# giladfrid009/WTracker

Hardware: AMD Instinct MI355X
Metric: frames/sec YOLOv8s+ResMLP sim loop @640x640 (higher is better)
Workload: dtype f16x3; 1 GPU; BASELINE configs[2]: full sim loop, YOLOv8s (nc=1, seeded synthetic weights) + ResMLP(imaging-100ms_pred-40ms_moving-50ms, reference weights); batch_per_gpu=64, lanes_per_gpu=2, global_batch=64, headline_mode=f16x3, parallelism=single GPU

## Files before the change

### wtracker_amd/_build.py

```python
from __future__ import annotations

import os
import subprocess
import sys

PKG_DIR = os.path.dirname(os.path.abspath(__file__))
CSRC = os.path.join(PKG_DIR, "csrc")
LIB_PATH = os.path.join(PKG_DIR, "libwtk_hip.so")
SOURCES = ["wtk_api.hip", "wtk_plan.hip", "wtk_run.hip", "wtk_hybrid.hip", "conv_igemm.hip", "conv_sk.hip", "conv1x1_wide.hip", "conv3x3_halo.hip", "conv3x3_c32.hip", "front_fused.hip", "front_fused_split.hip", "c2f_fused.hip", "stem_pool.hip", "head.hip", "mlp.hip", "track_ops.hip", "comm.hip", "eval_ops.hip"]
HEADERS = ["wtk_kernels.h", "wtk_internal.h", os.path.join("..", "..", "include", "wtk_hip.h")]


def _hipcc() -> str:
    for cand in (os.environ.get("HIPCC"), "/opt/rocm/bin/hipcc", "hipcc"):
        if cand and (os.path.isabs(cand) and os.path.exists(cand) or not os.path.isabs(cand)):
            return cand
    return "hipcc"


BASE_FLAGS = ["--offload-arch=gfx950", "-O3", "-fPIC", "-std=c++17", "-ffp-contract=off", "-Wall", "-Wno-unused-function"]
STAMP = os.path.join(CSRC, ".flags")


def _flags() -> list:
# ... 86 lines not shown
```

### wtracker_amd/csrc/conv3x3_halo.hip

```cpp
#include "wtk_kernels.h"

#include <cstdlib>
#include <type_traits>

namespace wtk {

typedef _Float16 half8 __attribute__((ext_vector_type(8)));
typedef float floatx4 __attribute__((ext_vector_type(4)));

namespace {

template <typename T> struct ElemH;
template <> struct ElemH<_Float16> {
    static constexpr int CE = 8;
};
template <> struct ElemH<float> {
    static constexpr int CE = 4;
};

__device__ __forceinline__ float silu_h(float x) {
    return wtk_silu_scaled(x);
}

__device__ __forceinline__ void mma_h(const uint4 &wf, const uint4 &pf, floatx4 &acc, _Float16 *) {
// ... 127 lines not shown
    const bool ok = halo_out_coords(a, o_first + lane, xs, n, y, x);
    col_e = xs + x;
    pix_e = ok ? (n * a.H + y) * a.W + col_e : -1;
}
__device__ __forceinline__ int lane_fetch(int src_lane, int v) { return __builtin_amdgcn_ds_bpermute(src_lane * 4, v); }

template <typename T, int BN, int NHALO, int MINW, int NWB, int HROWS, int BMT = 256, bool TAIL = false, bool SPLIT = false>
__global__ __launch_bounds__(512, MINW) void conv3x3_halo_kernel(const HaloArgs a) {
    static_assert(!SPLIT || (sizeof(T) == 2 && BN != 192 && (MINW <= 2 || (BN == 64 && BMT == 128 && NHALO == 1))),
                  "split mode: fp16 storage, 64 / 128 couts, 256-register budget (128 for the two-blocks-per-CU form: 64 couts x 128 pixels, one window buffer)");
#ifdef WTK_HALO_STAMPS
    const unsigned long long st_t0 = __builtin_amdgcn_s_memrealtime();
#endif
    asm volatile("" ::"s"(a.in), "s"(a.w), "s"(a.bias), "s"(a.zeros), "s"(a.in_ld), "s"(a.in_coff), "s"(a.N), "s"(a.H), "s"(a.W), "s"(a.Cin), "s"(a.CoutPad),
                 "s"(a.Kpad), "s"(a.S), "s"(a.pitch), "s"(a.strips), "s"(a.d_strips.mul), "s"(a.d_strips.sh1), "s"(a.d_strips.sh2), "s"(a.d_pitch.mul),
                 "s"(a.d_pitch.sh1), "s"(a.d_pitch.sh2), "s"(a.d_nct.mul), "s"(a.d_nct.sh1), "s"(a.d_nct.sh2), "s"(a.d_h1.mul), "s"(a.d_h1.sh1), "s"(a.d_h1.sh2), "s"(a.grid), "s"(a.live_off));
    constexpr int CE = ElemH<T>::CE;
    constexpr int CCH = 8 * CE;
    constexpr int WAVES_C = BN == 64 ? 1 : 2, WAVES_P = 8 / WAVES_C;
    constexpr int WC = BN / WAVES_C;
    constexpr int WP = BMT / WAVES_P, TP = WP / 16, TC = WC / 16, NV = 4 * TC;
    constexpr int WR = BN / 64;

    constexpr int kHaloBytesT = HROWS * 128;
    __shared__ __attribute__((aligned(16))) char halo0[kHaloBytesT];
    __shared__ __attribute__((aligned(16))) char halo1[NHALO == 2 ? kHaloBytesT : 16];
    static_assert(NWB == 2 || NWB == 3 || (NWB == 6 && NHALO == 2 && !TAIL && SPLIT), "slab ring: 2, 3 or 6 (split tiles, two window buffers, no fused tail)");
    constexpr bool kRing = NWB >= 3;
    __shared__ __attribute__((aligned(16))) char wbuf0[NWB > 3 ? 16 : BN * 128];
    __shared__ __attribute__((aligned(16))) char wbuf1[NWB > 3 ? 16 : BN * 128];
    __shared__ __attribute__((aligned(16))) char wbuf2[NWB == 3 ? BN * 128 : 16];
// ... 13 lines not shown
        if ((int)blockIdx.x >= live) return;
        nwg = min(nwg, live);
    }
    int L;
    {
        const int bid = blockIdx.x;
        const int xcd = bid & 7, q = nwg >> 3, r = nwg & 7;
        L = (xcd < r ? xcd * (q + 1) : r * (q + 1) + (xcd - r) * q) + (bid >> 3);
    }
    const unsigned t = fdiv((unsigned)L, a.d_nct);
    const int n0 = (L - (int)t * nct) * BN;
    const int rb = (int)fdiv(t, a.d_strips);
    const int strip = (int)t - rb * a.strips;
    const int o0 = rb * BMT;
    const char *zero_page = reinterpret_cast<const char *>(a.zeros);
    if (a.live_off) {
        const unsigned u = (unsigned)strip * (unsigned)a.live_ld + ((unsigned)o0 >> 7);
        const unsigned wd = *reinterpret_cast<const unsigned *>(zero_page + a.live_off + (u & ~3u));
        if (((wd >> ((u & 3u) * 8)) & (BMT == 256 ? 0xffffu : 0xffu)) == 0) return;
    }
    const int xs = strip * a.S;
    const int pitch = a.pitch;
    const int halo_rows = BMT + 2 * pitch + 2;
    const int halo_pieces = (halo_rows + 7) >> 3;
    const int n_base = (int)fdiv(fdiv((unsigned)o0, a.d_pitch), a.d_h1);

    const T *in = reinterpret_cast<const T *>(a.in) + (long long)n_base * a.H * a.W * a.in_ld + a.in_coff;
    const T *wgt = reinterpret_cast<const T *>(a.w);

    constexpr int kMaxPiecesPerWave = (HROWS / 8 + 7) / 8;
    unsigned hoff[kMaxPiecesPerWave];
    unsigned hvalid;
    halo_piece_offsets<T, kMaxPiecesPerWave>(a, o0, xs, n_base, halo_rows, wave, lane, hoff, hvalid);
    const char *img = reinterpret_cast<const char *>(in);
    auto issue_halo_piece = [&](char *buf, int q, int c) {
// ... 1442 lines not shown
    a.d_bps = make_fastdiv((unsigned)a.blocks_per_strip);
    a.d_strips = make_fastdiv((unsigned)a.strips);
    a.d_pitch = make_fastdiv((unsigned)a.pitch);
    a.d_h1 = make_fastdiv((unsigned)(a.H + 1));
    const long long cap = num_cus / 8 * 8;
    const unsigned grid = (unsigned)(tiles < cap ? tiles : cap);
    a.grid = (int)grid;
    hipLaunchKernelGGL((conv3x3_halo_pkernel<T, BN, HROWS>), dim3(grid), dim3(512), 0, stream, a);
    return hipGetLastError();
}

template <typename T, int BN, int NHALO, int MINW, int NWB, int HROWS, int BMT = 256, bool TAIL = false, bool SPLIT = false> hipError_t launch_h(HaloArgs a, hipStream_t stream) {
    const long long blocks = (long long)a.strips * a.blocks_per_strip * (a.CoutPad / BN);
    if (blocks <= 0 || blocks > 0x7fffffffLL) return hipErrorInvalidValue;
    if (BMT + 2 * a.pitch + 2 > HROWS || (long long)a.blocks_per_strip * BMT < (long long)a.N * (a.H + 1) * a.pitch) return hipErrorInvalidValue;
    if (a.live_off && ((a.live_off & 3u) || (a.live_ld & 1) || (long long)a.live_ld * 128 < (long long)a.blocks_per_strip * BMT)) return hipErrorInvalidValue;
    a.d_nct = make_fastdiv((unsigned)(a.CoutPad / BN));
    a.d_bps = make_fastdiv((unsigned)a.blocks_per_strip);
    a.d_strips = make_fastdiv((unsigned)a.strips);
    a.d_pitch = make_fastdiv((unsigned)a.pitch);
    a.d_h1 = make_fastdiv((unsigned)(a.H + 1));
    a.grid = (int)blocks;
    hipLaunchKernelGGL((conv3x3_halo_kernel<T, BN, NHALO, MINW, NWB, HROWS, BMT, TAIL, SPLIT>), dim3((unsigned)blocks), dim3(512), 0, stream, a);
    return hipGetLastError();
}

}

bool halo_eligible(int k, int stride, int cin, int is_f16) {
    const int cch = is_f16 ? 64 : 32;
    return k == 3 && stride == 1 && cin % cch == 0;
// ... 154 lines not shown
```

### wtracker_amd/csrc/head.hip

```cpp
#include "wtk_kernels.h"

namespace wtk {

template <typename T> __device__ __forceinline__ float ldf(const T *p) { return (float)*p; }

constexpr int kStatusNonFinite = 1;
__device__ __forceinline__ bool not_finite(float x) { return !(fabsf(x) <= 3.402823466e+38f); }

__device__ __forceinline__ void better(float &s, int &i, float s2, int i2) {
    if (s2 > s || (s2 == s && i2 < i)) {
        s = s2;
        i = i2;
    }
}

template <typename T>
__device__ __forceinline__ bool head_scan(const HeadArgs &a, int n, float &best, int &best_i, float &best_l, float &second) {
    const int A0 = a.lh[0] * a.lw[0], A1 = a.lh[1] * a.lw[1], A2 = a.lh[2] * a.lw[2];
    const int A = A0 + A1 + A2;

    best = -INFINITY, best_l = -INFINITY, second = -INFINITY;
    best_i = 0x7fffffff;
    bool bad = false;
    auto merge = [](float &b, int &bi, float &bl, float &s2nd, float b2, int bi2, float bl2, float s2) __attribute__((always_inline)) {
// ... 139 lines not shown
    head_row<T>(a, n, keep, best_i, score);
}

template <typename T>
__global__ __launch_bounds__(1024) void head_select_kernel_sparse(const HeadSparseArgs q) {
    const HeadArgs &a = q.h;
    const int n = blockIdx.x;
    float best, best_l, second;
    int best_i;
    if (!head_scan<T>(a, n, best, best_i, best_l, second)) return;
    if (threadIdx.x != 0) return;
    if (a.out_margin) a.out_margin[n] = fminf(best_l - second, fabsf(best_l - a.conf_logit));
    const bool keep = (best_i != 0x7fffffff) && (best > a.conf);
    q.sel_anchor[n] = keep ? best_i : -1;
    q.sel_score[n] = best;
    if (!keep || (q.n_dyn && n >= *q.n_dyn)) return;
    const int A0 = a.lh[0] * a.lw[0], A1 = a.lh[1] * a.lw[1];
    const int lvl = best_i < A0 ? 0 : (best_i < A0 + A1 ? 1 : 2);
    const int j = best_i - (lvl == 0 ? 0 : (lvl == 1 ? A0 : A0 + A1));
    const int H = a.lh[lvl], W = a.lw[lvl], S = q.S[lvl], pitch = q.pitch[lvl], ld = q.ld[lvl];
    const int y = j / W, x = j % W;
    unsigned char *live0 = q.live + q.off0[lvl], *live1 = q.live + q.off1[lvl];
    for (int dy = -1; dy <= 1; ++dy)
        for (int dx = -1; dx <= 1; ++dx) {
            const int yy = y + dy, xx = x + dx;
            if (yy < 0 || yy >= H || xx < 0 || xx >= W) continue;
            const int s = xx / S;
            const int u = s * ld + (((n * (H + 1) + yy) * pitch + (xx - s * S)) >> 7);
            live0[u] = 1;
            if (dy == 0 && dx == 0) live1[u] = 1;
        }
}

template <typename T>
__global__ __launch_bounds__(64) void head_decode_kernel(const HeadSparseArgs q) {
    const int n = blockIdx.x;
    const int best_i = q.sel_anchor[n];
    head_row<T>(q.h, n, best_i >= 0, best_i, q.sel_score[n]);
}

constexpr float kNmsMaxWh = 7680.f;

template <typename T> __device__ __forceinline__ void decode_anchor(const HeadArgs &a, int n, int lvl, int j, int Al, float (&xyxy)[4]) {
    const T *b = reinterpret_cast<const T *>(a.box[lvl]) + ((long long)n * Al + j) * 64;
    float dist[4];
#pragma unroll
// ... 133 lines not shown
    }
    if (threadIdx.x == 0 && q.out_count) q.out_count[n] = count;
}

hipError_t launch_head_nms(const NmsArgs &a, int is_f16, hipStream_t stream) {
    if (a.h.N <= 0 || a.h.nc < 1 || a.h.cls_ld < a.h.nc || a.max_det < 1 || !a.scratch_score || !a.scratch_cls || !a.scratch_box || !a.out_xywh)
        return hipErrorInvalidValue;
    if (is_f16)
        hipLaunchKernelGGL((head_nms_kernel<_Float16>), dim3(a.h.N), dim3(1024), 0, stream, a);
    else
        hipLaunchKernelGGL((head_nms_kernel<float>), dim3(a.h.N), dim3(1024), 0, stream, a);
    return hipGetLastError();
}

hipError_t launch_head_select_sparse(const HeadSparseArgs &a, hipStream_t stream) {
    if (a.h.N <= 0 || a.h.nc < 1 || a.h.cls_ld < a.h.nc || !a.live || !a.sel_anchor || !a.sel_score) return hipErrorInvalidValue;
    hipLaunchKernelGGL((head_select_kernel_sparse<float>), dim3(a.h.N), dim3(1024), 0, stream, a);
    return hipGetLastError();
}
hipError_t launch_head_decode(const HeadSparseArgs &a, hipStream_t stream) {
    if (a.h.N <= 0 || !a.sel_anchor || !a.sel_score || !a.h.out_xywh) return hipErrorInvalidValue;
    hipLaunchKernelGGL((head_decode_kernel<float>), dim3(a.h.N), dim3(64), 0, stream, a);
    return hipGetLastError();
}

hipError_t launch_head(const HeadArgs &a, int is_f16, hipStream_t stream) {
    if (a.N <= 0 || a.nc < 1 || a.cls_ld < a.nc) return hipErrorInvalidValue;
    if (is_f16)
        hipLaunchKernelGGL((head_select_kernel<_Float16>), dim3(a.N), dim3(1024), 0, stream, a);
    else
        hipLaunchKernelGGL((head_select_kernel<float>), dim3(a.N), dim3(1024), 0, stream, a);
// ... 5 lines not shown
```

### wtracker_amd/csrc/wtk_internal.h

```cpp
#pragma once
#include "../../include/wtk_hip.h"
#include "wtk_kernels.h"

#include <cstring>
#include <map>
#include <mutex>
#include <string>
#include <utility>
#include <vector>

namespace wtk {
int fail(const std::string &msg);
int fail_hip(const char *what, hipError_t e);
int ensure_attributes(int device);
}
#define HIP_TRY(expr)                                                                                                          \
    do {                                                                                                                       \
        hipError_t _e = (expr);                                                                                                \
        if (_e != hipSuccess) return wtk::fail_hip(#expr, _e);                                                                 \
    } while (0)

struct DeviceGuard {
    int prev = -1;
    bool switched = false;
// ... 123 lines not shown
    int *nms_cls = nullptr;
    int use_halo = 1;
    int front_debug = 0;
    int use_tail = 1;
    int use_tail_cls_split = 1;
    int halo_small_blocks = 1;
    int halo_persist = 1;
    int halo_slabs = 3;
    int use_c32s = 1;
    int use_s2win = 1;
    int use_ws64 = 1;
    int use_wide = 1;
    int use_c2f = 0;
    int use_front = 0;
    int use_sparse_box = 1;
    struct DetLevel {
        int op0 = -1, box1 = -1, box2 = -1;
    } det[3];
    size_t live_bytes = 0;
    int *sel_anchor = nullptr;
    float *sel_score = nullptr;
    int sparse_B = 0;
    ConvLaunch sparse_done[6];
    int num_cus = 0;
    int latency = 0;
    int sk_group = 1;
    int sk_force_tile = -1, sk_force_form = -1;
    std::map<long long, wtk::SkChoice> sk_choices;
    int sk_autotune = 1;
    int tune_pass = -1;
    std::map<long long, std::vector<wtk::SkChoice>> sk_cands;
    std::map<long long, std::vector<float>> tune_ms;
    std::vector<hipEvent_t> tune_ev;
    std::vector<long long> tune_key;
// ... 31 lines not shown
```

### wtracker_amd/csrc/wtk_kernels.h

```cpp
#pragma once
#include <hip/hip_runtime.h>
#include <stdint.h>

namespace wtk {

struct FastDiv {
    unsigned mul, sh1, sh2;
};
inline FastDiv make_fastdiv(unsigned d) {
    FastDiv f;
    if (d == 0) d = 1;
    unsigned l = 0;
    while ((1ull << l) < d) ++l;
    const unsigned long long m = ((1ull << 32) * ((1ull << l) - d)) / d + 1;
    f.mul = (unsigned)m;
    f.sh1 = l < 1 ? l : 1;
    f.sh2 = l > 0 ? l - 1 : 0;
    return f;
}
__device__ __forceinline__ unsigned fdiv(unsigned n, const FastDiv &f) {
    const unsigned t = __umulhi(n, f.mul);
    return (t + ((n - t) >> f.sh1)) >> f.sh2;
}

// ... 197 lines not shown
    int S, pitch, strips, blocks_per_strip;
    const void *zeros;
    unsigned long long *dbg_stamps;
    const void *tail_w;
    const float *tail_bias;
    void *tail_out;
    int tail_kpad, tail_ld, tail_coff;
    int tail_cout;
    int tail_f32;
    int bm;
    int persist_cus;
    int slabs;
    int deep;
    int narrow;
    int grid;
    unsigned live_off;
    const int *n_dyn;
    FastDiv d_bps, d_strips, d_pitch, d_nct, d_h1;
    int live_ld;
};
static_assert(sizeof(HaloArgs) == 288, "live_off / live_ld fill padding: the struct of a dense launch is what it was before the live mask");
bool halo_eligible(int k, int stride, int cin, int is_f16);
bool split_halo_eligible(int k, int stride, int cin, int cout);
int split_halo_cout_tile(int cout_stored);
hipError_t launch_conv3x3_halo_split(const HaloArgs &a, hipStream_t stream);
bool split_s2win_eligible(int k, int stride, int cin, int cout, int cout_pad, int wo, bool plain);
hipError_t launch_conv3x3_s2_split(const HaloArgs &a, hipStream_t stream);
int halo_rows_max(int cout_stored, int slabs);
void halo_geometry(int H, int W, int rows_max, int *S, int *pitch, int *strips, int *blocks_per_strip, int bm = 256);
void halo_geometry_stacked(int N, int H, int W, int rows_max, int *S, int *pitch, int *strips, int *blocks_per_strip, int bm = 256);
int halo_cout_tile(int cout_stored);
hipError_t launch_conv3x3_halo(const HaloArgs &a, int is_f16, hipStream_t stream);
bool s2win_eligible(int k, int stride, int cin, int cout, int cout_pad, int is_f16, int wo, bool plain);
hipError_t launch_conv3x3_s2(const HaloArgs &a, hipStream_t stream);
int ws64_rows_max();
bool ws64_eligible(int k, int stride, int cin, int cout, int cout_pad, int is_f16, bool has_out2, bool has_tail);
// ... 115 lines not shown
    int N;
    float conf;
    float gain, pad_x, pad_y;
    float img_w, img_h;
    float *out_xywh;
    float *out_conf;
    int *out_anchor;
    float *out_margin;
    float conf_logit;
    int *status;
};
hipError_t launch_head(const HeadArgs &a, int is_f16, hipStream_t stream);

struct HeadSparseArgs {
    HeadArgs h;
    unsigned char *live;
    int *sel_anchor;
    float *sel_score;
    int S[3], pitch[3], ld[3];
    unsigned off0[3], off1[3];
    const int *n_dyn;
};
hipError_t launch_head_select_sparse(const HeadSparseArgs &a, hipStream_t stream);
hipError_t launch_head_decode(const HeadSparseArgs &a, hipStream_t stream);

struct NmsArgs {
    HeadArgs h;
    float iou;
    int max_det;
    float *scratch_score;
    int *scratch_cls;
    float *scratch_box;
    float *out_xywh;
    float *out_conf;
    int *out_cls;
    int *out_anchor;
    int *out_count;
};
hipError_t launch_head_nms(const NmsArgs &a, int is_f16, hipStream_t stream);
// ... 111 lines not shown
```

### wtracker_amd/csrc/wtk_plan.hip

```cpp
#include <execinfo.h>
#include <signal.h>
#include <unistd.h>

#include "wtk_internal.h"

#include <algorithm>
#include <cmath>
#include <cstdio>
#include <cstdlib>

using namespace wtk;

namespace {
static int make_divisible8(double x) { return (int)(std::ceil(x / 8.0) * 8.0); }

static ModelDims model_dims(float width, float depth, int max_ch, int nc) {
    ModelDims d;
    const int base[5] = {64, 128, 256, 512, 1024};
    for (int i = 0; i < 5; ++i) d.c[i] = make_divisible8(std::min(base[i], max_ch) * (double)width);
    const int nb[4] = {3, 6, 6, 3};
    for (int i = 0; i < 4; ++i) d.n[i] = std::max((int)std::lround(nb[i] * (double)depth), 1);
    d.hb = std::max(std::max(16, d.c[2] / 4), 64);
    d.hc = std::max(d.c[2], std::min(nc, 100));
    d.nc = nc;
// ... 311 lines not shown
    h->halo_persist = env_int("WTK_HALO_PERSIST", 1) != 0;
    h->halo_small_blocks = env_int("WTK_HALO_SMALL_BLOCKS", 1) != 0;
    h->use_tail = env_int("WTK_NO_FUSED_TAIL", 0) != 1;
    h->use_tail_cls_split = env_int("WTK_NO_SPLIT_CLS_TAIL", 0) != 1;
    h->use_wide = env_int("WTK_NO_WIDE_1X1", 0) != 1;
    h->use_ws64 = env_int("WTK_NO_WS64", 0) != 1;
    h->use_s2win = env_int("WTK_NO_S2WIN", 0) != 1;
    h->use_c32s = env_int("WTK_NO_C32S", 0) != 1;
    h->sk_group = env_int("WTK_SK_GROUP", 1) != 0;
    h->sk_autotune = env_int("WTK_SK_AUTOTUNE", 1) != 0;
    const int tile = env_int("WTK_SK_TILE", -1), form = env_int("WTK_SK_FORM", -1);
    h->sk_force_tile = tile >= 0 && tile <= 3 ? tile : -1;
    h->sk_force_form = form == 0 || form == 1 ? form : -1;
    h->front_debug = env_int("WTK_FRONT_DEBUG", 0) == 1;
    h->use_sparse_box = env_int("WTK_NO_SPARSE_BOX", 0) != 1;
    PlanSwitches s;
    s.latency_plan = env_int("WTK_LATENCY_PLAN", -1);
    s.no_side_stream = env_int("WTK_NO_SIDE_STREAM", 0) == 1;
    s.materialize_upsample = env_int("WTK_MATERIALIZE_UPSAMPLE", 0) == 1;
    s.no_igemm_tail = env_int("WTK_NO_IGEMM_TAIL", 0) == 1;
    s.no_sk_mixed = env_int("WTK_NO_SK_MIXED", 0) == 1;
    s.small_narrow = env_int("WTK_SMALL_NARROW", 1) != 0;
    s.halo_deep = env_int("WTK_HALO_DEEP", 1);
    s.sk_finish = env_int("WTK_SK_FINISH", 0) == 1;
    s.no_fused_front = env_int("WTK_NO_FUSED_FRONT", 0) == 1;
    s.no_fused_c2f = env_int("WTK_NO_FUSED_C2F", 0) == 1;
    return s;
}
}

// ... 417 lines not shown
            wtk_yolo_destroy(h);
            return 1;
        }
    }
    if (dev_alloc(h, (void **)&h->o_xywh, sizeof(float) * 4 * h->max_batch) || dev_alloc(h, (void **)&h->o_conf, sizeof(float) * h->max_batch) ||
        dev_alloc(h, (void **)&h->o_anchor, sizeof(int) * h->max_batch) || dev_alloc(h, (void **)&h->o_margin, sizeof(float) * h->max_batch)) {
        wtk_yolo_destroy(h);
        return 1;
    }
    if (acquire_status_word(&h->status_host, &h->status_dev)) {
        h->status_host = nullptr;
        wtk_yolo_destroy(h);
        return fail("wtk_yolo_create: no pinned status word (hipHostMalloc failed, or more than 4096 live handles)");
    }
    if (h->split && !h->latency && h->use_sparse_box && wtk::sparse_box_pays(h->max_batch, h->lh[0], h->lw[0], h->num_cus)) {
        size_t total = 0;
        for (int i = 0; i < 3; ++i) {
            int S, pitch, strips, bps;
            halo_geometry_stacked(h->max_batch, h->lh[i], h->lw[i], kHaloRowsMax, &S, &pitch, &strips, &bps, 256);
            total += 2 * (((size_t)strips * 2 * bps + 3) & ~(size_t)3);
        }
        h->live_bytes = total;
        if (dev_alloc(h, (void **)&h->sel_anchor, sizeof(int) * h->max_batch) || dev_alloc(h, (void **)&h->sel_score, sizeof(float) * h->max_batch)) {
            wtk_yolo_destroy(h);
            return 1;
        }
    }
    if (dev_alloc(h, &h->zero_page, 256 + h->live_bytes)) {
        wtk_yolo_destroy(h);
        return 1;
    }
    if (hipMemset(h->zero_page, 0, 256 + h->live_bytes) != hipSuccess) {
        wtk_yolo_destroy(h);
        return fail("wtk_yolo_create: hipMemset failed");
    }
    *out = h;
    return 0;
}

extern "C" int wtk_yolo_status(wtk_yolo *h, int32_t *flags, int32_t clear) {
    if (!h || !flags) return fail("wtk_yolo_status: null argument");
    *flags = h->status_static | (h->status_host ? __atomic_load_n(h->status_host, __ATOMIC_RELAXED) : 0);
    if (clear && h->status_host) __atomic_store_n(h->status_host, 0, __ATOMIC_RELAXED);
    return 0;
}

extern "C" int wtk_yolo_workload(wtk_yolo *h, double *macs_per_frame, int32_t *anchors) {
// ... 39 lines not shown
```

### wtracker_amd/csrc/wtk_run.hip

```cpp
#include "wtk_internal.h"

#include <algorithm>
#include <cmath>
#include <cstdio>
#include <cstdlib>

using namespace wtk;

#ifdef WTK_WS64_STAMPS
static unsigned long long *g_dbg_stamps = nullptr;
constexpr size_t kDbgStampBytes = 1 << 20;
extern "C" int wtk_debug_stamps(unsigned long long *host, size_t n_words) {
    if (!g_dbg_stamps || n_words * 8 > kDbgStampBytes) return 1;
    if (hipDeviceSynchronize() != hipSuccess) return 1;
    return hipMemcpy(host, g_dbg_stamps, n_words * 8, hipMemcpyDeviceToHost) == hipSuccess ? 0 : 1;
}
#endif

static void letterbox_geom(int H, int W, int Sh, int Sw, int &new_h, int &new_w, int &top, int &left, float &gain, float &pad_x, float &pad_y) {
    const double r = std::min((double)Sh / H, (double)Sw / W);
    new_w = (int)std::nearbyint(W * r);
    new_h = (int)std::nearbyint(H * r);
    const double dw = (Sw - new_w) / 2.0, dh = (Sh - new_h) / 2.0;
    top = (int)std::nearbyint(dh - 0.1);
// ... 213 lines not shown
    } else if (h->use_s2win && op.tail_op < 0 && s2win_eligible(op.k, op.stride, op.cin, op.cout, op.cout_pad, h->is_f16, ob.w, plain) && halves) {
        r.kind = L_S2WIN;
        r.g = s2win_args(h, op, a);
    } else if (op.tail_op >= 0) {
        const Op &t = h->ops[op.tail_op];
        a.tail_w = t.w, a.tail_bias = t.bias, a.tail_kpad = t.Kpad, a.tail_act = t.act;
        a.tail_out = h->bufs[t.out_buf].ptr, a.tail_ld = h->bufs[t.out_buf].C, a.tail_coff = t.out_coff;
    } else if (h->use_wide && conv1x1_wide_eligible(a, h->is_f16) && a.CoutPad >= 256 && ((a.M + 255) / 256) * (a.CoutPad / 128) >= 384) {
        r.kind = L_WIDE_1X1;
    }
    return 0;
}

struct SparseBox {
    ConvLaunch cls0[3], box0[3], box1[3];
    HeadSparseArgs hs;
    int level_of_op0(const wtk_yolo *h, size_t oi) const {
        for (int l = 0; l < 3; ++l)
            if ((int)oi == h->det[l].op0) return l;
        return -1;
    }
    bool skips(const wtk_yolo *h, size_t oi) const {
        for (int l = 0; l < 3; ++l)
            if ((int)oi == h->det[l].box1 || (int)oi == h->det[l].box2) return true;
        return false;
    }
};

static bool resolve_sparse(const wtk_yolo *h, int B, SparseBox &sp) {
    if (!h->use_sparse_box || !h->split || h->latency || !h->live_bytes) return false;
    if (!sparse_box_pays(B, h->lh[0], h->lw[0], h->num_cus)) return false;
    std::memset(&sp.hs, 0, sizeof(sp.hs));
    unsigned off = 0;
    for (int l = 0; l < 3; ++l) {
        const wtk_yolo::DetLevel &d = h->det[l];
        if (d.op0 < 0 || d.box1 < 0 || d.box2 < 0) return false;
        const Op &o0 = h->ops[d.op0], &b1 = h->ops[d.box1], &b2 = h->ops[d.box2];
        if (o0.folded || o0.tail_op >= 0 || o0.cout != h->dims.hb + h->dims.hc || h->dims.hb != 64 || h->dims.hc % 64 || b1.tail_op != d.box2 || !b2.folded) return false;
        ConvLaunch r0, r1;
        if (resolve_conv(h, o0, B, r0) || resolve_conv(h, b1, B, r1)) return false;
        if (r0.kind != L_HALO_SPLIT || r1.kind != L_HALO_SPLIT || r0.g.res || r0.g.out2 || r1.g.res || r1.g.out2) return false;
        if (split_halo_cout_tile(o0.cout) != 64 || r0.g.narrow || r1.g.narrow) return false;
        if (r0.g.S != r1.g.S || r0.g.pitch != r1.g.pitch || r0.g.strips != r1.g.strips) return false;
        const int ld = 2 * (int)(((long long)B * (h->lh[l] + 1) * r0.g.pitch + 255) / 256);
        const unsigned bytes = ((unsigned)r0.g.strips * (unsigned)ld + 3u) & ~3u;
        sp.hs.S[l] = r0.g.S, sp.hs.pitch[l] = r0.g.pitch, sp.hs.ld[l] = ld;
        sp.hs.off0[l] = off, sp.hs.off1[l] = off + bytes;
        off += 2 * bytes;
        if (off > h->live_bytes) return false;
        const int hb = h->dims.hb;
        sp.box0[l] = r0;
        sp.box0[l].g.Cout = sp.box0[l].g.CoutPad = hb;
        sp.box0[l].g.live_off = 256u + sp.hs.off0[l], sp.box0[l].g.live_ld = ld;
        sp.cls0[l] = r0;
        HaloArgs &c = sp.cls0[l].g;
        c.Cout = c.CoutPad = o0.cout - hb, c.narrow = 1;
        c.w = reinterpret_cast<const char *>(c.w) + (size_t)hb * c.Kpad * 2;
        c.bias = c.bias + hb;
        c.out_coff += 2 * hb;
        sp.box1[l] = r1;
        sp.box1[l].g.live_off = 256u + sp.hs.off1[l], sp.box1[l].g.live_ld = ld;
    }
    sp.hs.live = reinterpret_cast<unsigned char *>(h->zero_page) + 256;
    sp.hs.sel_anchor = h->sel_anchor, sp.hs.sel_score = h->sel_score, sp.hs.n_dyn = h->n_dyn;
    return true;
}

constexpr long long kOpKeyBase = 100000;
static long long choice_key(long long launch, int B) { return (launch << 24) | (long long)B; }

static int issue_conv(wtk_yolo *h, const Op &op, const ConvLaunch &r, hipStream_t st) {
    switch (r.kind) {
    case L_IGEMM: HIP_TRY(launch_conv(r.a, r.cfg, h->is_f16, st)); break;
    case L_IGEMM_SPLIT: HIP_TRY(launch_conv_split(r.a, r.cfg, st)); break;
    case L_WIDE_1X1: HIP_TRY(launch_conv1x1_wide(r.a, st)); break;
    case L_HALO: HIP_TRY(launch_conv3x3_halo(r.g, h->is_f16, st)); break;
    case L_HALO_SPLIT: HIP_TRY(launch_conv3x3_halo_split(r.g, st)); break;
    case L_C32: HIP_TRY(launch_conv3x3_c32(r.g, st)); break;
    case L_C32_SPLIT: HIP_TRY(launch_conv3x3_c32_split(r.g, st)); break;
// ... 198 lines not shown
            HIP_TRY(hipEventRecord(ev[0], p.main_st));
        }
        HIP_TRY(launch_conv_sk_group(m, n, h->split, h->num_cus, h->sk_force_tile, h->sk_force_form, p.main_st, choice));
        if (ev) {
            HIP_TRY(hipEventRecord(ev[1], p.main_st));
            h->tune_key[li] = key;
        }
        p.count(PROF_IGEMM);
    }
    return 0;
}

static int enqueue_sparse_tail(Pass &p, const SparseBox &sp, int H, int W, float conf, float *out_xywh, float *out_conf, int *out_anchor) {
    wtk_yolo *h = p.h;
    hipStream_t st = p.main_st;
    HeadSparseArgs hs = sp.hs;
    hs.h = head_args(h, p.B, H, W, conf, out_xywh, out_conf, out_anchor);
    if (mark(p, PROF_HEAD)) return 1;
    HIP_TRY(hipMemsetAsync(hs.live, 0, h->live_bytes, st));
    HIP_TRY(launch_head_select_sparse(hs, st));
    p.count(PROF_HEAD);
    if (mark(p, PROF_SPARSE)) return 1;
    for (int l = 0; l < 3; ++l) {
        if (issue_conv(h, h->ops[h->det[l].op0], sp.box0[l], st)) return 1;
        p.count(PROF_SPARSE);
    }
    for (int l = 0; l < 3; ++l) {
        if (issue_conv(h, h->ops[h->det[l].box1], sp.box1[l], st)) return 1;
        p.count(PROF_SPARSE);
    }
    if (mark(p, PROF_HEAD)) return 1;
    HIP_TRY(launch_head_decode(hs, st));
    p.count(PROF_HEAD);
    h->sparse_B = p.B;
    for (int l = 0; l < 3; ++l) {
        h->sparse_done[l] = sp.box0[l], h->sparse_done[3 + l] = sp.box1[l];
        h->sparse_done[l].g.live_off = h->sparse_done[3 + l].g.live_off = 0;
        h->sparse_done[l].g.live_ld = h->sparse_done[3 + l].g.live_ld = 0;
    }
    return 0;
}

static int complete_box_towers(wtk_yolo *h) {
    if (!h->sparse_B) return 0;
    for (int l = 0; l < 3; ++l)
        if (issue_conv(h, h->ops[h->det[l].op0], h->sparse_done[l], nullptr)) return 1;
    for (int l = 0; l < 3; ++l)
        if (issue_conv(h, h->ops[h->det[l].box1], h->sparse_done[3 + l], nullptr)) return 1;
    HIP_TRY(hipDeviceSynchronize());
    h->sparse_B = 0;
    return 0;
}

static int yolo_enqueue_pass(wtk_yolo *h, const uint8_t *frames_dev, int32_t B, int32_t H, int32_t W, int32_t C, float conf, float *out_xywh,
                             float *out_conf, int32_t *out_anchor, hipStream_t st, const ViewSrc *vs, const NmsOut *nms) {
    Pass p{h, frames_dev, B, C, st};
    SparseBox sp;
    if (!nms && resolve_sparse(h, B, sp)) {
        hipStreamCaptureStatus cs = hipStreamCaptureStatusNone;
// ... 343 lines not shown
```

Before: 11550 frames/s.

## Replace live-mask sparse box tower with per-frame box patch kernels

Drops the live-mask scheme, in which the head marked halo tiles around each frame's selected anchor and the full halo conv launches skipped dead tiles. A dedicated box_patch kernel now computes the 3x3 neighbourhood of the selected anchor per frame directly with MFMA, and a second stage fuses the box1 conv with its 1x1 tail at the centre pixel. This removes the live-mask memset, the mask writes and the large mostly-empty halo grids. The cost is a new hand-written kernel with fixed channel assumptions (Cin multiple of 64, Cin of 128 in the tail stage) that must match the dense results.

After: 11650 frames/s (median of 6 runs). Within noise of the previous version (+0.9%).

```diff
diff --git a/wtracker_amd/_build.py b/wtracker_amd/_build.py
--- a/wtracker_amd/_build.py
+++ b/wtracker_amd/_build.py
@@ -7,7 +7,7 @@
 PKG_DIR = os.path.dirname(os.path.abspath(__file__))
 CSRC = os.path.join(PKG_DIR, "csrc")
 LIB_PATH = os.path.join(PKG_DIR, "libwtk_hip.so")
-SOURCES = ["wtk_api.hip", "wtk_plan.hip", "wtk_run.hip", "wtk_hybrid.hip", "conv_igemm.hip", "conv_sk.hip", "conv1x1_wide.hip", "conv3x3_halo.hip", "conv3x3_c32.hip", "front_fused.hip", "front_fused_split.hip", "c2f_fused.hip", "stem_pool.hip", "head.hip", "mlp.hip", "track_ops.hip", "comm.hip", "eval_ops.hip"]
+SOURCES = ["wtk_api.hip", "wtk_plan.hip", "wtk_run.hip", "wtk_hybrid.hip", "conv_igemm.hip", "conv_sk.hip", "conv1x1_wide.hip", "conv3x3_halo.hip", "conv3x3_c32.hip", "box_patch.hip", "front_fused.hip", "front_fused_split.hip", "c2f_fused.hip", "stem_pool.hip", "head.hip", "mlp.hip", "track_ops.hip", "comm.hip", "eval_ops.hip"]
 HEADERS = ["wtk_kernels.h", "wtk_internal.h", os.path.join("..", "..", "include", "wtk_hip.h")]
 
 
diff --git a/wtracker_amd/csrc/box_patch.hip b/wtracker_amd/csrc/box_patch.hip
--- /dev/null
+++ b/wtracker_amd/csrc/box_patch.hip
@@ -0,0 +1,137 @@
+#include "wtk_kernels.h"
+
+namespace wtk {
+
+namespace {
+
+typedef _Float16 half8 __attribute__((ext_vector_type(8)));
+typedef _Float16 half4 __attribute__((ext_vector_type(4)));
+typedef float floatx4 __attribute__((ext_vector_type(4)));
+
+struct TapFrag {
+    half8 wh, wl, ph, pl;
+};
+
+template <bool TAIL>
+__global__ __launch_bounds__(256) void box_patch_kernel(const BoxPatchArgs a) {
+    const int n = blockIdx.x;
+    if (a.n_dyn && n >= *a.n_dyn) return;
+    const int j = a.sel_anchor[n] - a.anchor0;
+    if (j < 0 || j >= a.H * a.W) return;
+    const int y = j / a.W, x = j - y * a.W;
+
+    const int lane = threadIdx.x & 63, wave = __builtin_amdgcn_readfirstlane(threadIdx.x >> 6);
+    const int lr = lane & 15, lg = lane >> 4;
+    const int oy = TAIL ? y : y + lr / 3 - 1, ox = TAIL ? x : x + lr % 3 - 1;
+    const bool live = (TAIL ? lr == 0 : lr < 9) && oy >= 0 && oy < a.H && ox >= 0 && ox < a.W;
+    unsigned tap_ok = 0;
+#pragma unroll
+    for (int t = 0; t < 9; ++t) {
+        const int iy = oy + t / 3 - 1, ix = ox + t % 3 - 1;
+        tap_ok |= (live && iy >= 0 && iy < a.H && ix >= 0 && ix < a.W) ? 1u << t : 0u;
+    }
+    const long long pix = ((long long)n * a.H + (live ? oy : y)) * a.W + (live ? ox : x);
+    const _Float16 *pin = reinterpret_cast<const _Float16 *>(a.in) + pix * a.in_ld + a.in_coff + lg * 8;
+    const int wrow = (lr >> 2) * 16 + 4 * wave + (lr & 3);
+    const _Float16 *pw = reinterpret_cast<const _Float16 *>(a.w) + (long long)wrow * a.Kpad + lg * 8;
+
+    const int groups = 3 * (a.Cin / 64);
+    auto load_group = [&](TapFrag(&f)[3], int g) __attribute__((always_inline)) {
+        g = min(g, groups - 1);
+        const int c = g / 3, kh = g - 3 * c;
+#pragma unroll
+        for (int kw = 0; kw < 3; ++kw) {
+            const int t = kh * 3 + kw;
+            const _Float16 *w = pw + (long long)t * a.Cin + c * 64;
+            f[kw].wh = *reinterpret_cast<const half8 *>(w);
+            f[kw].wl = *reinterpret_cast<const half8 *>(w + 32);
+            const _Float16 *p = ((tap_ok >> t) & 1u) ? pin + (long long)((kh - 1) * a.W + (kw - 1)) * a.in_ld + c * 64 : reinterpret_cast<const _Float16 *>(a.zeros);
+            f[kw].ph = *reinterpret_cast<const half8 *>(p);
+            f[kw].pl = *reinterpret_cast<const half8 *>(p + 32);
+        }
+    };
+    const int cb = lg * 16 + 4 * wave;
+    floatx4 acc = {a.bias[cb], a.bias[cb + 1], a.bias[cb + 2], a.bias[cb + 3]}, acc1 = {0.f, 0.f, 0.f, 0.f};
+    auto mma_group = [&](const TapFrag(&f)[3]) __attribute__((always_inline)) {
+#pragma unroll
+        for (int kw = 0; kw < 3; ++kw) {
+            acc = __builtin_amdgcn_mfma_f32_16x16x32_f16(f[kw].wh, f[kw].ph, acc, 0, 0, 0);
+            acc1 = __builtin_amdgcn_mfma_f32_16x16x32_f16(f[kw].wl, f[kw].ph, acc1, 0, 0, 0);
+            acc1 = __builtin_amdgcn_mfma_f32_16x16x32_f16(f[kw].wh, f[kw].pl, acc1, 0, 0, 0);
+        }
+    };
+    TapFrag f0[3], f1[3], f2[3];
+    load_group(f0, 0);
+    load_group(f1, 1);
+    for (int g = 0; g < groups; g += 3) {
+        load_group(f2, g + 2);
+        mma_group(f0);
+        load_group(f0, g + 3);
+        mma_group(f1);
+        load_group(f1, g + 4);
+        mma_group(f2);
+    }
+
+    float v[4];
+#pragma unroll
+    for (int r = 0; r < 4; ++r) v[r] = wtk_split_value(acc[r], acc1[r]);
+    if (a.act) wtk_silu_scaled_run<4>(v);
+    half4 hv, lv;
+#pragma unroll
+    for (int r = 0; r < 4; ++r) {
+        const _Float16 h = (_Float16)v[r];
+        hv[r] = h;
+        lv[r] = (_Float16)((v[r] - (float)h) * kSplitScale);
+    }
+    if constexpr (!TAIL) {
+        if (!live) return;
+        _Float16 *p = reinterpret_cast<_Float16 *>(a.out) + pix * a.out_ld + a.out_coff + 64 * (cb >> 5) + (cb & 31);
+        *reinterpret_cast<half4 *>(p) = hv;
+        *reinterpret_cast<half4 *>(p + 32) = lv;
+    } else {
+        __shared__ __attribute__((aligned(16))) _Float16 tile[2][16][64];
+        {
+            _Float16 *q = &tile[cb >> 5][lr][cb & 31];
+            *reinterpret_cast<half4 *>(q) = hv;
+            *reinterpret_cast<half4 *>(q + 32) = lv;
+        }
+        const _Float16 *w2 = reinterpret_cast<const _Float16 *>(a.tail_w) + (long long)wrow * a.tail_kpad + lg * 8;
+        half8 wh2[2], wl2[2];
+#pragma unroll
+        for (int blk = 0; blk < 2; ++blk) {
+            wh2[blk] = *reinterpret_cast<const half8 *>(w2 + blk * 64);
+            wl2[blk] = *reinterpret_cast<const half8 *>(w2 + blk * 64 + 32);
+        }
+        floatx4 acc2 = {a.tail_bias[cb], a.tail_bias[cb + 1], a.tail_bias[cb + 2], a.tail_bias[cb + 3]}, acc2l = {0.f, 0.f, 0.f, 0.f};
+        __syncthreads();
+#pragma unroll
+        for (int blk = 0; blk < 2; ++blk) {
+            const half8 ph = *reinterpret_cast<const half8 *>(&tile[blk][lr][lg * 8]);
+            const half8 pl = *reinterpret_cast<const half8 *>(&tile[blk][lr][32 + lg * 8]);
+            acc2 = __builtin_amdgcn_mfma_f32_16x16x32_f16(wh2[blk], ph, acc2, 0, 0, 0);
+            acc2l = __builtin_amdgcn_mfma_f32_16x16x32_f16(wl2[blk], ph, acc2l, 0, 0, 0);
+            acc2l = __builtin_amdgcn_mfma_f32_16x16x32_f16(wh2[blk], pl, acc2l, 0, 0, 0);
+        }
+        if (!live) return;
+        float *o = reinterpret_cast<float *>(a.tail_out) + pix * a.tail_ld + a.tail_coff + cb;
+        *reinterpret_cast<float4 *>(o) = make_float4(wtk_split_value(acc2[0], acc2l[0]), wtk_split_value(acc2[1], acc2l[1]), wtk_split_value(acc2[2], acc2l[2]),
+                                                     wtk_split_value(acc2[3], acc2l[3]));
+    }
+}
+
+}
+
+hipError_t launch_box_patch(const BoxPatchArgs &a, int stage, hipStream_t stream) {
+    if (a.N <= 0 || a.H <= 0 || a.W <= 0 || !a.in || !a.w || !a.bias || !a.zeros || !a.sel_anchor || a.anchor0 < 0) return hipErrorInvalidValue;
+    if (a.Cin <= 0 || a.Cin % 64 || a.Kpad != 9 * a.Cin || a.in_ld % 64 || a.in_coff % 64 || a.in_coff + a.Cin > a.in_ld) return hipErrorInvalidValue;
+    if (stage == 0) {
+        if (!a.out || a.out_ld % 64 || a.out_coff % 64 || a.out_coff + 128 > a.out_ld) return hipErrorInvalidValue;
+        hipLaunchKernelGGL((box_patch_kernel<false>), dim3((unsigned)a.N), dim3(256), 0, stream, a);
+    } else {
+        if (a.Cin != 128 || !a.tail_w || !a.tail_bias || !a.tail_out || a.tail_kpad != 128 || a.tail_ld % 4 || a.tail_coff % 4 || a.tail_coff + 64 > a.tail_ld) return hipErrorInvalidValue;
+        hipLaunchKernelGGL((box_patch_kernel<true>), dim3((unsigned)a.N), dim3(256), 0, stream, a);
+    }
+    return hipGetLastError();
+}
+
+}
diff --git a/wtracker_amd/csrc/conv3x3_halo.hip b/wtracker_amd/csrc/conv3x3_halo.hip
--- a/wtracker_amd/csrc/conv3x3_halo.hip
+++ b/wtracker_amd/csrc/conv3x3_halo.hip
@@ -165,7 +165,7 @@
 #endif
     asm volatile("" ::"s"(a.in), "s"(a.w), "s"(a.bias), "s"(a.zeros), "s"(a.in_ld), "s"(a.in_coff), "s"(a.N), "s"(a.H), "s"(a.W), "s"(a.Cin), "s"(a.CoutPad),
                  "s"(a.Kpad), "s"(a.S), "s"(a.pitch), "s"(a.strips), "s"(a.d_strips.mul), "s"(a.d_strips.sh1), "s"(a.d_strips.sh2), "s"(a.d_pitch.mul),
-                 "s"(a.d_pitch.sh1), "s"(a.d_pitch.sh2), "s"(a.d_nct.mul), "s"(a.d_nct.sh1), "s"(a.d_nct.sh2), "s"(a.d_h1.mul), "s"(a.d_h1.sh1), "s"(a.d_h1.sh2), "s"(a.grid), "s"(a.live_off));
+                 "s"(a.d_pitch.sh1), "s"(a.d_pitch.sh2), "s"(a.d_nct.mul), "s"(a.d_nct.sh1), "s"(a.d_nct.sh2), "s"(a.d_h1.mul), "s"(a.d_h1.sh1), "s"(a.d_h1.sh2), "s"(a.grid));
     constexpr int CE = ElemH<T>::CE;
     constexpr int CCH = 8 * CE;
     constexpr int WAVES_C = BN == 64 ? 1 : 2, WAVES_P = 8 / WAVES_C;
@@ -209,11 +209,6 @@
     const int strip = (int)t - rb * a.strips;
     const int o0 = rb * BMT;
     const char *zero_page = reinterpret_cast<const char *>(a.zeros);
-    if (a.live_off) {
-        const unsigned u = (unsigned)strip * (unsigned)a.live_ld + ((unsigned)o0 >> 7);
-        const unsigned wd = *reinterpret_cast<const unsigned *>(zero_page + a.live_off + (u & ~3u));
-        if (((wd >> ((u & 3u) * 8)) & (BMT == 256 ? 0xffffu : 0xffu)) == 0) return;
-    }
     const int xs = strip * a.S;
     const int pitch = a.pitch;
     const int halo_rows = BMT + 2 * pitch + 2;
@@ -1686,7 +1681,6 @@
     const long long blocks = (long long)a.strips * a.blocks_per_strip * (a.CoutPad / BN);
     if (blocks <= 0 || blocks > 0x7fffffffLL) return hipErrorInvalidValue;
     if (BMT + 2 * a.pitch + 2 > HROWS || (long long)a.blocks_per_strip * BMT < (long long)a.N * (a.H + 1) * a.pitch) return hipErrorInvalidValue;
-    if (a.live_off && ((a.live_off & 3u) || (a.live_ld & 1) || (long long)a.live_ld * 128 < (long long)a.blocks_per_strip * BMT)) return hipErrorInvalidValue;
     a.d_nct = make_fastdiv((unsigned)(a.CoutPad / BN));
     a.d_bps = make_fastdiv((unsigned)a.blocks_per_strip);
     a.d_strips = make_fastdiv((unsigned)a.strips);
diff --git a/wtracker_amd/csrc/head.hip b/wtracker_amd/csrc/head.hip
--- a/wtracker_amd/csrc/head.hip
+++ b/wtracker_amd/csrc/head.hip
@@ -177,22 +177,6 @@
     const bool keep = (best_i != 0x7fffffff) && (best > a.conf);
     q.sel_anchor[n] = keep ? best_i : -1;
     q.sel_score[n] = best;
-    if (!keep || (q.n_dyn && n >= *q.n_dyn)) return;
-    const int A0 = a.lh[0] * a.lw[0], A1 = a.lh[1] * a.lw[1];
-    const int lvl = best_i < A0 ? 0 : (best_i < A0 + A1 ? 1 : 2);
-    const int j = best_i - (lvl == 0 ? 0 : (lvl == 1 ? A0 : A0 + A1));
-    const int H = a.lh[lvl], W = a.lw[lvl], S = q.S[lvl], pitch = q.pitch[lvl], ld = q.ld[lvl];
-    const int y = j / W, x = j % W;
-    unsigned char *live0 = q.live + q.off0[lvl], *live1 = q.live + q.off1[lvl];
-    for (int dy = -1; dy <= 1; ++dy)
-        for (int dx = -1; dx <= 1; ++dx) {
-            const int yy = y + dy, xx = x + dx;
-            if (yy < 0 || yy >= H || xx < 0 || xx >= W) continue;
-            const int s = xx / S;
-            const int u = s * ld + (((n * (H + 1) + yy) * pitch + (xx - s * S)) >> 7);
-            live0[u] = 1;
-            if (dy == 0 && dx == 0) live1[u] = 1;
-        }
 }
 
 template <typename T>
@@ -356,7 +340,7 @@
 }
 
 hipError_t launch_head_select_sparse(const HeadSparseArgs &a, hipStream_t stream) {
-    if (a.h.N <= 0 || a.h.nc < 1 || a.h.cls_ld < a.h.nc || !a.live || !a.sel_anchor || !a.sel_score) return hipErrorInvalidValue;
+    if (a.h.N <= 0 || a.h.nc < 1 || a.h.cls_ld < a.h.nc || !a.sel_anchor || !a.sel_score) return hipErrorInvalidValue;
     hipLaunchKernelGGL((head_select_kernel_sparse<float>), dim3(a.h.N), dim3(1024), 0, stream, a);
     return hipGetLastError();
 }
diff --git a/wtracker_amd/csrc/wtk_internal.h b/wtracker_amd/csrc/wtk_internal.h
--- a/wtracker_amd/csrc/wtk_internal.h
+++ b/wtracker_amd/csrc/wtk_internal.h
@@ -161,10 +161,10 @@
     int use_c2f = 0;
     int use_front = 0;
     int use_sparse_box = 1;
+    int sparse_debug = 0;
     struct DetLevel {
         int op0 = -1, box1 = -1, box2 = -1;
     } det[3];
-    size_t live_bytes = 0;
     int *sel_anchor = nullptr;
     float *sel_score = nullptr;
     int sparse_B = 0;
diff --git a/wtracker_amd/csrc/wtk_kernels.h b/wtracker_amd/csrc/wtk_kernels.h
--- a/wtracker_amd/csrc/wtk_kernels.h
+++ b/wtracker_amd/csrc/wtk_kernels.h
@@ -235,12 +235,10 @@
     int deep;
     int narrow;
     int grid;
-    unsigned live_off;
     const int *n_dyn;
     FastDiv d_bps, d_strips, d_pitch, d_nct, d_h1;
-    int live_ld;
-};
-static_assert(sizeof(HaloArgs) == 288, "live_off / live_ld fill padding: the struct of a dense launch is what it was before the live mask");
+};
+static_assert(sizeof(HaloArgs) == 288, "the launch trace of tests/hostsan hashes the argument bytes: keep the layout");
 bool halo_eligible(int k, int stride, int cin, int is_f16);
 bool split_halo_eligible(int k, int stride, int cin, int cout);
 int split_halo_cout_tile(int cout_stored);
@@ -386,15 +384,31 @@
 
 struct HeadSparseArgs {
     HeadArgs h;
-    unsigned char *live;
     int *sel_anchor;
     float *sel_score;
-    int S[3], pitch[3], ld[3];
-    unsigned off0[3], off1[3];
-    const int *n_dyn;
 };
 hipError_t launch_head_select_sparse(const HeadSparseArgs &a, hipStream_t stream);
 hipError_t launch_head_decode(const HeadSparseArgs &a, hipStream_t stream);
+
+struct BoxPatchArgs {
+    const void *in;
+    int in_ld, in_coff;
+    int N, H, W, Cin;
+    const void *w;
+    const float *bias;
+    int Kpad, act;
+    const void *zeros;
+    void *out;
+    int out_ld, out_coff;
+    const void *tail_w;
+    const float *tail_bias;
+    void *tail_out;
+    int tail_kpad, tail_ld, tail_coff;
+    const int *sel_anchor;
+    int anchor0;
+    const int *n_dyn;
+};
+hipError_t launch_box_patch(const BoxPatchArgs &a, int stage, hipStream_t stream);
 
 struct NmsArgs {
     HeadArgs h;
diff --git a/wtracker_amd/csrc/wtk_plan.hip b/wtracker_amd/csrc/wtk_plan.hip
--- a/wtracker_amd/csrc/wtk_plan.hip
+++ b/wtracker_amd/csrc/wtk_plan.hip
@@ -349,6 +349,7 @@
     h->sk_force_form = form == 0 || form == 1 ? form : -1;
     h->front_debug = env_int("WTK_FRONT_DEBUG", 0) == 1;
     h->use_sparse_box = env_int("WTK_NO_SPARSE_BOX", 0) != 1;
+    h->sparse_debug = env_int("WTK_SPARSE_BOX_DEBUG", 0) == 1;
     PlanSwitches s;
     s.latency_plan = env_int("WTK_LATENCY_PLAN", -1);
     s.no_side_stream = env_int("WTK_NO_SIDE_STREAM", 0) == 1;
@@ -796,23 +797,16 @@
         return fail("wtk_yolo_create: no pinned status word (hipHostMalloc failed, or more than 4096 live handles)");
     }
     if (h->split && !h->latency && h->use_sparse_box && wtk::sparse_box_pays(h->max_batch, h->lh[0], h->lw[0], h->num_cus)) {
-        size_t total = 0;
-        for (int i = 0; i < 3; ++i) {
-            int S, pitch, strips, bps;
-            halo_geometry_stacked(h->max_batch, h->lh[i], h->lw[i], kHaloRowsMax, &S, &pitch, &strips, &bps, 256);
-            total += 2 * (((size_t)strips * 2 * bps + 3) & ~(size_t)3);
-        }
-        h->live_bytes = total;
         if (dev_alloc(h, (void **)&h->sel_anchor, sizeof(int) * h->max_batch) || dev_alloc(h, (void **)&h->sel_score, sizeof(float) * h->max_batch)) {
             wtk_yolo_destroy(h);
             return 1;
         }
     }
-    if (dev_alloc(h, &h->zero_page, 256 + h->live_bytes)) {
+    if (dev_alloc(h, &h->zero_page, 256)) {
         wtk_yolo_destroy(h);
         return 1;
     }
-    if (hipMemset(h->zero_page, 0, 256 + h->live_bytes) != hipSuccess) {
+    if (hipMemset(h->zero_page, 0, 256) != hipSuccess) {
         wtk_yolo_destroy(h);
         return fail("wtk_yolo_create: hipMemset failed");
     }
diff --git a/wtracker_amd/csrc/wtk_run.hip b/wtracker_amd/csrc/wtk_run.hip
--- a/wtracker_amd/csrc/wtk_run.hip
+++ b/wtracker_amd/csrc/wtk_run.hip
@@ -251,7 +251,7 @@
 
 struct SparseBox {
     ConvLaunch cls0[3], box0[3], box1[3];
-    HeadSparseArgs hs;
+    BoxPatchArgs patch0[3], patch1[3];
     int level_of_op0(const wtk_yolo *h, size_t oi) const {
         for (int l = 0; l < 3; ++l)
             if ((int)oi == h->det[l].op0) return l;
@@ -264,11 +264,23 @@
     }
 };
 
+static BoxPatchArgs patch_args(const wtk_yolo *h, const HaloArgs &g, int anchor0) {
+    BoxPatchArgs q;
+    std::memset(&q, 0, sizeof(q));
+    q.in = g.in, q.in_ld = g.in_ld, q.in_coff = g.in_coff;
+    q.N = g.N, q.H = g.H, q.W = g.W, q.Cin = g.Cin;
+    q.w = g.w, q.bias = g.bias, q.Kpad = g.Kpad, q.act = g.act, q.zeros = h->zero_page;
+    q.out = g.out, q.out_ld = g.out_ld, q.out_coff = g.out_coff;
+    q.tail_w = g.tail_w, q.tail_bias = g.tail_bias, q.tail_out = g.tail_out;
+    q.tail_kpad = g.tail_kpad, q.tail_ld = g.tail_ld, q.tail_coff = g.tail_coff;
+    q.sel_anchor = h->sel_anchor, q.anchor0 = anchor0, q.n_dyn = h->n_dyn;
+    return q;
+}
+
 static bool resolve_sparse(const wtk_yolo *h, int B, SparseBox &sp) {
-    if (!h->use_sparse_box || !h->split || h->latency || !h->live_bytes) return false;
+    if (!h->use_sparse_box || !h->split || h->latency || !h->sel_anchor) return false;
     if (!sparse_box_pays(B, h->lh[0], h->lw[0], h->num_cus)) return false;
-    std::memset(&sp.hs, 0, sizeof(sp.hs));
-    unsigned off = 0;
+    int anchor0 = 0;
     for (int l = 0; l < 3; ++l) {
         const wtk_yolo::DetLevel &d = h->det[l];
         if (d.op0 < 0 || d.box1 < 0 || d.box2 < 0) return false;
@@ -278,17 +290,10 @@
         if (resolve_conv(h, o0, B, r0) || resolve_conv(h, b1, B, r1)) return false;
         if (r0.kind != L_HALO_SPLIT || r1.kind != L_HALO_SPLIT || r0.g.res || r0.g.out2 || r1.g.res || r1.g.out2) return false;
         if (split_halo_cout_tile(o0.cout) != 64 || r0.g.narrow || r1.g.narrow) return false;
-        if (r0.g.S != r1.g.S || r0.g.pitch != r1.g.pitch || r0.g.strips != r1.g.strips) return false;
-        const int ld = 2 * (int)(((long long)B * (h->lh[l] + 1) * r0.g.pitch + 255) / 256);
-        const unsigned bytes = ((unsigned)r0.g.strips * (unsigned)ld + 3u) & ~3u;
-        sp.hs.S[l] = r0.g.S, sp.hs.pitch[l] = r0.g.pitch, sp.hs.ld[l] = ld;
-        sp.hs.off0[l] = off, sp.hs.off1[l] = off + bytes;
-        off += 2 * bytes;
-        if (off > h->live_bytes) return false;
+        if (r0.g.H != h->lh[l] || r0.g.W != h->lw[l] || r1.g.H != h->lh[l] || r1.g.W != h->lw[l] || !r1.g.tail_f32 || r1.g.tail_cout != 64) return false;
         const int hb = h->dims.hb;
         sp.box0[l] = r0;
         sp.box0[l].g.Cout = sp.box0[l].g.CoutPad = hb;
-        sp.box0[l].g.live_off = 256u + sp.hs.off0[l], sp.box0[l].g.live_ld = ld;
         sp.cls0[l] = r0;
         HaloArgs &c = sp.cls0[l].g;
         c.Cout = c.CoutPad = o0.cout - hb, c.narrow = 1;
@@ -296,10 +301,10 @@
         c.bias = c.bias + hb;
         c.out_coff += 2 * hb;
         sp.box1[l] = r1;
-        sp.box1[l].g.live_off = 256u + sp.hs.off1[l], sp.box1[l].g.live_ld = ld;
-    }
-    sp.hs.live = reinterpret_cast<unsigned char *>(h->zero_page) + 256;
-    sp.hs.sel_anchor = h->sel_anchor, sp.hs.sel_score = h->sel_score, sp.hs.n_dyn = h->n_dyn;
+        sp.patch0[l] = patch_args(h, sp.box0[l].g, anchor0);
+        sp.patch1[l] = patch_args(h, sp.box1[l].g, anchor0);
+        anchor0 += h->lh[l] * h->lw[l];
+    }
     return true;
 }
 
@@ -528,35 +533,32 @@
 static int enqueue_sparse_tail(Pass &p, const SparseBox &sp, int H, int W, float conf, float *out_xywh, float *out_conf, int *out_anchor) {
     wtk_yolo *h = p.h;
     hipStream_t st = p.main_st;
-    HeadSparseArgs hs = sp.hs;
+    HeadSparseArgs hs;
+    std::memset(&hs, 0, sizeof(hs));
     hs.h = head_args(h, p.B, H, W, conf, out_xywh, out_conf, out_anchor);
+    hs.sel_anchor = h->sel_anchor, hs.sel_score = h->sel_score;
     if (mark(p, PROF_HEAD)) return 1;
-    HIP_TRY(hipMemsetAsync(hs.live, 0, h->live_bytes, st));
     HIP_TRY(launch_head_select_sparse(hs, st));
     p.count(PROF_HEAD);
     if (mark(p, PROF_SPARSE)) return 1;
     for (int l = 0; l < 3; ++l) {
-        if (issue_conv(h, h->ops[h->det[l].op0], sp.box0[l], st)) return 1;
+        HIP_TRY(launch_box_patch(sp.patch0[l], 0, st));
         p.count(PROF_SPARSE);
     }
     for (int l = 0; l < 3; ++l) {
-        if (issue_conv(h, h->ops[h->det[l].box1], sp.box1[l], st)) return 1;
+        HIP_TRY(launch_box_patch(sp.patch1[l], 1, st));
         p.count(PROF_SPARSE);
     }
     if (mark(p, PROF_HEAD)) return 1;
     HIP_TRY(launch_head_decode(hs, st));
     p.count(PROF_HEAD);
     h->sparse_B = p.B;
-    for (int l = 0; l < 3; ++l) {
-        h->sparse_done[l] = sp.box0[l], h->sparse_done[3 + l] = sp.box1[l];
-        h->sparse_done[l].g.live_off = h->sparse_done[3 + l].g.live_off = 0;
-        h->sparse_done[l].g.live_ld = h->sparse_done[3 + l].g.live_ld = 0;
-    }
+    for (int l = 0; l < 3; ++l) h->sparse_done[l] = sp.box0[l], h->sparse_done[3 + l] = sp.box1[l];
     return 0;
 }
 
 static int complete_box_towers(wtk_yolo *h) {
-    if (!h->sparse_B) return 0;
+    if (!h->sparse_B || h->sparse_debug) return 0;
     for (int l = 0; l < 3; ++l)
         if (issue_conv(h, h->ops[h->det[l].op0], h->sparse_done[l], nullptr)) return 1;
     for (int l = 0; l < 3; ++l)
```
